# JuliaRobotics/KernelDensityEstimate.jl

Hardware: AMD Instinct MI355X
Metric: gibbs_product_samples_per_sec (higher is better)
Workload: dtype f64

## Files before the change

kerneldensityestimate.jl_amd/csrc/gibbs_lean.hip:

```cpp
#define KDEHIP_EXP256 1
#ifndef KDEHIP_PRELOAD_MAXB
#define KDEHIP_PRELOAD_MAXB 8
#endif
#include "gibbs_device.hpp"
#include "screen_device.hpp"

namespace kdehip {

template <int I> using IC = std::integral_constant<int, I>;
template <int N, int I = 0, typename F>
__device__ __forceinline__ void static_for(F &&f) {
  if constexpr (I < N) {
    f(IC<I>{});
    static_for<N, I + 1>(f);
  }
}

#if defined(KDEHIP_LEAN_HI) || (defined(KDEHIP_LEAN_DEV_M) && KDEHIP_LEAN_DEV_M > 4)
constexpr int kLeanMinDens = 8, kLeanMaxDens = 8;
#else
constexpr int kLeanMinDens = 2, kLeanMaxDens = 4;
#endif
constexpr int kLeanMaxNormals = 128;

__device__ __forceinline__ int scalar_copy(int x) {
  int y;
  asm("s_mov_b32 %0, %1" : "=s"(y) : "s"(x));
  return y;
}

template <int D>
struct LeanTile {
  int n;
  int flags;
  int lds_off;
  int stage_bytes;
  int chunk_rows;
  int seg;
  int hdr_lo, hdr_hi;
  int B, F, last_lane;
  int uniform_bw;
  __device__ __forceinline__ int64_t hdr_off() const {
    return (static_cast<int64_t>(hdr_hi) << 32) | static_cast<uint32_t>(hdr_lo);
  }
  __device__ __forceinline__ void load(const kdehip_v8i &d) {
    n = scalar_copy(d[0]);
    flags = scalar_copy(d[1]);
    lds_off = scalar_copy(d[2]);
    stage_bytes = scalar_copy(d[3]);
    chunk_rows = scalar_copy(d[4]);
    seg = scalar_copy(d[5]);
    hdr_lo = scalar_copy(d[6]);
    hdr_hi = scalar_copy(d[7]);
    B = (n + 63) >> 6;
    last_lane = flags & 0xFF;
    uniform_bw = flags >> 8;
    F = uniform_bw ? D + 1 : 2 * D + 1;
  }
};

template <typename P, typename T, bool OK> constexpr bool kCanPreloadImpl = OK && kIsLdsPtr<P> && sizeof(T) == 8;

template <typename T, int D, int M, int WAVES, bool BATCH = false, bool SCHUNK = false>
__global__ __launch_bounds__(WAVES * 64) void gibbs_lean_kernel(PlanDev plan_, RunArgs a_) {
  const LaunchView<BATCH> view(plan_, a_);
  const PlanDev &plan = view.plan;
  const auto &a = view.a;
  constexpr bool kPrefetchRows = (WAVES <= 12) || sizeof(T) == 4 || D <= 4;
  using RowPtr = std::conditional_t<(WAVES == 16 && sizeof(T) == 8), LdsPtrSplit<T>, LdsPtr<T>>;
  constexpr int kCopyWaves = WAVES > 4 ? 4 : WAVES;
  constexpr bool kKeptRows = (WAVES <= 8);
  constexpr bool kScreen = sizeof(T) == 8 && !BATCH;
  constexpr bool kPreloadBuild = kKeptRows && kPrefetchRows;
  constexpr int kNormOff = 2048;
  constexpr int kUnifOff = kNormOff + WAVES * kLeanMaxNormals * 8;
  constexpr int kPoolOff = kUnifOff + WAVES * 1024;
  constexpr bool kCoop = kScreen && SCHUNK && WAVES == 8;
  constexpr int kXchgOff = kPoolOff + kLdsPoolBytes;
  constexpr int kXchgSlotDoubles = 32 + 4 * 64;
  constexpr int kXchgBytes = kCoop ? 64 + WAVES * kXchgSlotDoubles * 8 : 0;
  static_assert(kPoolOff + kLdsPoolBytes + kXchgBytes <= 160 * 1024, "LDS budget of one CU exceeded");
  __shared__ __attribute__((aligned(1024))) unsigned char smem[kPoolOff + kLdsPoolBytes + kXchgBytes];

  double *sExpTab = reinterpret_cast<double *>(smem);
  if (threadIdx.x < 256) sExpTab[threadIdx.x] = kExp2Tab256[threadIdx.x];
  if constexpr (kCoop) {
    if (threadIdx.x < 16) reinterpret_cast<int *>(smem + kXchgOff)[threadIdx.x] = 0;
  }

  const int lane = threadIdx.x & 63;
  const int wave = __builtin_amdgcn_readfirstlane(static_cast<int>(threadIdx.x >> 6));
  KDEHIP_PRIO_CHAIN();
  const int chain = wave;
  int64_t s = static_cast<int64_t>(view.block) * WAVES + chain;
  const bool live = s < a.Np;
  if (!live) s = a.Np - 1;
  const uint64_t gs = static_cast<uint64_t>(a.sample_offset + s);
  const void *fb = live ? static_cast<const void *>(plan.levels) : nullptr;

  const int L = plan.L;
  const T *__restrict__ data = static_cast<const T *>(plan.data);
  const LevelTable levels{(const __attribute__((address_space(4))) kdehip_v16i *)(plan.levels)};
  const StepTable steps{(const __attribute__((address_space(4))) kdehip_v8i *)(plan.levels + 2 * plan.M * (plan.L + 1))};
  unsigned char *pool = smem + kPoolOff;
  const int dl = lane < D ? lane : D - 1;
  const int vlev = a.variant % 1000;

  double *sNorm = reinterpret_cast<double *>(smem + kNormOff) + chain * kLeanMaxNormals;
  const int R = D * (L + 1);
  if (a.rng_philox) {
    for (int b = lane; 2 * b < R; b += 64) {
      double n0, n1;
      philox_normal_pair(a.seed, gs, static_cast<uint32_t>(b), n0, n1);
      sNorm[2 * b] = n0;
      if (2 * b + 1 < R) sNorm[2 * b + 1] = n1;
    }
  } else {
    for (int r = lane; r < R; r += 64) sNorm[r] = a.randN[s * a.R + r];
  }
  __syncthreads();

  T lam[M], lmu[M];
  int psel[M];

  auto adopt = [&](auto jc, const auto &ds, auto hdr, int pos) {
    constexpr int j = decltype(jc)::value;
    using TA = TileAddr<T>;
    auto e = hdr + kTileHeader + TA::row(pos >> 6, TA::stride(ds.F)) + (pos & 63) * TA::kLane;
    const T mu = e[dl * TA::kField];
    const T var = ds.uniform_bw ? hdr[dl] : e[(D + dl) * TA::kField];
    const T l = fast_rcp(var);
    lam[j] = l;
    lmu[j] = mu * l;
    psel[j] = pos;
  };
  auto product = [&](auto skipc, T &mean, T &cov) {
    constexpr int skip = decltype(skipc)::value;
    T ls = T(0), ms = T(0);
    static_for<M>([&](auto kc) {
      constexpr int k = decltype(kc)::value;
      if constexpr (k != skip) { ls += lam[k]; ms += lmu[k]; }
    });
    cov = fast_rcp(ls);
    mean = cov * ms;
  };

  auto draw = [&](const auto &ds, auto hdr, T mean, T cov, auto &&run) -> int {
    if (ds.uniform_bw) {
      EvalUniform<T, D> ev;
      ev.tab = sExpTab;
      const T c = hdr[dl] + cov;
      T cen, nin;
      EvalUniform<T, D>::operands(mean, c, true, cen, nin);
      T Pr = T(1);
#pragma unroll
      for (int d = 0; d < D; ++d) {
        ev.center[d] = lane_read(cen, d);
        ev.ninv[d] = lane_read(nin, d);
        Pr *= lane_read(c, d);
      }
      ev.scale = Num<T>::rsqrt(Pr);
      return run(ev);
    }
    EvalFast<T, D, false> ev;
    ev.tab = sExpTab;
    ev.act = 0;
#pragma unroll
    for (int d = 0; d < D; ++d) {
      ev.center[d] = lane_read(mean, d);
      ev.cov[d] = lane_read(cov, d);
    }
    return run(ev);
  };

  uint32_t c = static_cast<uint32_t>(M);
  uint32_t ubatch = 0xFFFFFFFFu;
  double *sUnif = reinterpret_cast<double *>(smem + kUnifOff) + wave * 128;
  auto next_uniform = [&]() -> double {
    const uint32_t b = c >> 7;
    if (b != ubatch) {
      ubatch = b;
      double u_even, u_odd;
      if (a.rng_philox) {
        const Philox4 r = philox_block(a.seed, gs, b * 64u + static_cast<uint32_t>(lane), 0u);
        u_even = bits_to_unit(r.v[0], r.v[1]);
        u_odd = bits_to_unit(r.v[2], r.v[3]);
      } else {
        const int64_t i0 = s * a.K + static_cast<int64_t>(b) * 128 + 2 * lane - 1;
        u_even = (i0 >= 0 && i0 < a.nU) ? a.randU[i0] : 0.5;
        u_odd = (i0 + 1 < a.nU) ? a.randU[i0 + 1] : 0.5;
      }
      wave_sync();
      sUnif[2 * lane] = u_even;
      sUnif[2 * lane + 1] = u_odd;
      wave_sync();
    }
    const double u = sUnif[c & 127u];
    ++c;
    return u;
  };

  static_for<M>([&](auto jc) {
    const LevelDesc ds = levels[decltype(jc)::value * (L + 1)];
    adopt(jc, ds, data + ds.hdr_off, 0);
  });

  const TabTable tabs{(const __attribute__((address_space(4))) kdehip_v8i *)(plan.tabdesc)};
  const T *tables = static_cast<const T *>(plan.tables);
  const int Lt = (vlev == 1 || vlev == 4 || !a.use_tables) ? 0 : plan.Lt;

  auto draw_rows = [&](const auto &ds, auto rows, const auto &ev, double u) -> int {
    using P = decltype(rows);
    return draw_label<T, P, kPrefetchRows, kKeptRows>(rows, ds, lane, ev, u, fb);
  };

  auto draw_rows_repeat = [&](const auto &ds, const T *rows, const auto &ev, double u) -> int {
    using Ev = std::decay_t<decltype(ev)>;
    if constexpr (kScreen && SCHUNK && sizeof(typename Ev::Row) <= 7 * sizeof(T) && WAVES <= 8) {
      LaneAcc<T> acc;
      KDEHIP_PRIO_ROWS();
      lane_rows_all_deep<T, Ev>(rows, ds.B, TileAddr<T>::stride(ds.F), lane, ev, acc);
      KDEHIP_PRIO_CHAIN();
      return select_or_raise<T, const T *>(acc.total(), rows, ds, lane, ev, u, fb);
    }
    return draw_rows(ds, rows, ev, u);
  };

#ifdef KDEHIP_SCREEN_STAMPS
  unsigned long long rstamp[8] = {0, 0, 0, 0, 0, 0, 0, 0}, r_prev_end = 0;
  bool rstamp_on = false;
#define RSTAMP(var) const unsigned long long var = __builtin_amdgcn_s_memtime()
#define RSTAMP_ADD(slot, t0, t1) do { if (rstamp_on) rstamp[slot] += (t1) - (t0); } while (0)
#else
#define RSTAMP(var) do {} while (0)
#define RSTAMP_ADD(slot, t0, t1) do {} while (0)
#endif
  auto step_kept = [&](auto jc, const auto &ds, auto hdr, const auto &row, T mean, T cov, double u) {
    RSTAMP(tr1);
    auto rows1 = hdr + kTileHeader;
    using P1 = decltype(rows1);
    using Ev = EvalFast<T, D, false>;
    Ev ev;
    ev.tab = sExpTab;
    ev.act = 0;
#pragma unroll
    for (int d = 0; d < D; ++d) {
      ev.center[d] = lane_read(mean, d);
      ev.cov[d] = lane_read(cov, d);
    }
#ifdef KDEHIP_SCREEN_STAMPS
    asm volatile("" ::"s"(ev.center[D - 1]), "s"(ev.cov[D - 1]));
#endif
    RSTAMP(tr2);
    RSTAMP_ADD(1, tr1, tr2);
    int pos1;
    if (ds.B == 1) {
      const T S = ev(row);
      pos1 = select_or_raise<T, P1>(S, rows1, ds, lane, ev, u, fb);
    } else if (ds.B <= 4) {
      pos1 = draw_label_kept<T, P1, Ev, 4>(rows1, ds, lane, ev, u, fb, row);
    } else {
      pos1 = draw_label_kept<T, P1, Ev, 8>(rows1, ds, lane, ev, u, fb, row);
    }
    pos1 = __builtin_amdgcn_readfirstlane(pos1);
    RSTAMP(tr3);
    RSTAMP_ADD(2, tr2, tr3);
    adopt(jc, ds, hdr, pos1);
#ifdef KDEHIP_SCREEN_STAMPS
    {
      const double sink = lam[decltype(jc)::value] + lmu[decltype(jc)::value];
      asm volatile("" ::"v"(sink));
    }
#endif
    RSTAMP(tr4);
    RSTAMP_ADD(3, tr3, tr4);
#ifdef KDEHIP_SCREEN_STAMPS
    r_prev_end = tr4;
#endif
  };

  auto step = [&](auto jc, const auto &ds, auto hdr, bool first, T x) {
    if constexpr (kCanPreloadImpl<decltype(hdr + kTileHeader), T, kPreloadBuild>) {
      if (!ds.uniform_bw && ds.B <= KDEHIP_PRELOAD_MAXB) {
        RSTAMP(tr0);
#ifdef KDEHIP_SCREEN_STAMPS
        if (r_prev_end) RSTAMP_ADD(4, r_prev_end, tr0);
#endif
        const auto row = EvalFast<T, D, false>().load(hdr + kTileHeader + lane * TileAddr<T>::kLane);
        T mean1 = x, cov1 = T(0);
        if (!first) product(jc, mean1, cov1);
        const double u1 = next_uniform();
#ifdef KDEHIP_SCREEN_STAMPS
        asm volatile("" ::"v"(mean1), "v"(cov1), "v"(u1));
        {
          RSTAMP(trp);
          RSTAMP_ADD(0, tr0, trp);
        }
#endif
        step_kept(jc, ds, hdr, row, mean1, cov1, u1);
        return;
      }
    }
    T mean = x, cov = T(0);
    if (!first) product(jc, mean, cov);
    const double u = next_uniform();
    auto rows = hdr + kTileHeader;
    const int pos = __builtin_amdgcn_readfirstlane(draw(ds, hdr, mean, cov, [&](const auto &ev) {
      return draw_rows(ds, rows, ev, u);
    }));
    adopt(jc, ds, hdr, pos);
  };

  uint32_t n_screened = 0, n_repeated = 0;
#ifdef KDEHIP_SCREEN_STAMPS
  unsigned long long sstamp[8] = {0, 0, 0, 0, 0, 0, 0, 0};
  bool sstamp_on = false;
#endif
  auto screen_eval = [&](const auto &ds, double mu0, double cmin, float mmax, float valid, T mean, T cov, auto &&body) -> int {
    const float cen = static_cast<float>(mean - mu0);
    const float cf = static_cast<float>(cmin + cov), covf = static_cast<float>(cov);
    const float acen = fabsf(cen);
    const float t = fminf(mmax + acen, 2.0f * acen);
    float a2 = lane < D ? t * t * __builtin_amdgcn_rcpf(cf) : 0.0f;
    const bool inr = (acen <= kScreenMaxAbsMean) && (covf <= static_cast<float>(kScreenMaxVar)) && (a2 <= kScreenMaxA2);
    const bool ok = valid != 0.0f && __ballot(lane < D && !inr) == 0ull;
    a2 += dpp_fetch<0x111, 0xF>(a2);
    a2 += dpp_fetch<0x112, 0xF>(a2);
    a2 += dpp_fetch<0x114, 0xF>(a2);
    const float na = __builtin_sqrtf(lane_read(a2, 7)) * (kScreenU * kScreenSqrtC0 * 1.01f);
    using SC = ScreenConst<D>;
    const float Bc = (kScreenLn2 * 1.01f) * (na + (ds.uniform_bw ? SC::kx_uni : SC::kx_node) * kScreenU);
    const float A = (kScreenLn2 * 1.01f) * na +
                    (static_cast<float>(((ds.B + 1) >> 1) + 9) + (ds.uniform_bw ? SC::vc_uni : SC::vc_node)) * kScreenU;
    if (ds.uniform_bw) {
      ScreenEval<D, true> ev;
      ev.A = A; ev.Bc = Bc;
      const float ninv = -kScreenC0 * __builtin_amdgcn_rcpf(cf);
      float pr = 1.0f;
#pragma unroll
      for (int d = 0; d < D; ++d) {
        ev.cen[d] = lane_read(cen, d);
        ev.b[d] = lane_read(ninv, d);
        pr *= lane_read(cf, d);
      }
      ev.scale = __builtin_amdgcn_rsqf(pr);
      return body(ev, ok);
    } else {
      ScreenEval<D, false> ev;
      ev.A = A; ev.Bc = Bc; ev.scale = 1.0f;
#pragma unroll
      for (int d = 0; d < D; ++d) {
        ev.cen[d] = lane_read(cen, d);
        ev.b[d] = lane_read(covf, d);
      }
      return body(ev, ok);
    }
  };
  auto screen_finish = [&](auto jc, const auto &ds, int pos, T mean, T cov, double u) {
    const T *hdrg = data + ds.hdr_off();
    ++n_screened;
    if (pos < 0) {
      ++n_repeated;
      pos = __builtin_amdgcn_readfirstlane(draw(ds, hdrg, mean, cov, [&](const auto &ev) {
        return draw_rows_repeat(ds, hdrg + kTileHeader, ev, u);
      }));
    }
    adopt(jc, ds, hdrg, pos);
  };
  bool pend = false;
  T pend_mean = T(0), pend_cov = T(0);
  double pend_u = 0.0;
  int cstep = 0;
  auto coop_post = [&](T mean, T cov, double u) {
    if constexpr (kCoop) {
      pend = true; pend_mean = mean; pend_cov = cov; pend_u = u;
      double *xs = reinterpret_cast<double *>(smem + kXchgOff + 64) + wave * kXchgSlotDoubles;
      if (lane < D) { xs[dl] = static_cast<double>(mean); xs[8 + dl] = static_cast<double>(cov); }
      if (lane == 0) reinterpret_cast<int *>(smem + kXchgOff)[(cstep & 1) * WAVES + wave] = 1;
    }
  };
  auto coop_resolve = [&](auto jp, const auto &dsp, int par) {
    if constexpr (kCoop) {
      int *flags = reinterpret_cast<int *>(smem + kXchgOff) + par * WAVES;
      const int f = flags[lane & (WAVES - 1)];
      const unsigned mask = static_cast<unsigned>(__ballot(f != 0 && lane < WAVES));
      if (mask == 0u) return;
      using TA = TileAddr<T>;
      const T *hdrg = data + dsp.hdr_off();
      const T *rows = hdrg + kTileHeader;
      const int RS = TA::stride(dsp.F), B = dsp.B;
      const int group = wave >> 2, k = wave & 3;
      int idx = 0;
      for (unsigned m = mask; m != 0u; m &= m - 1u, ++idx) {
        if ((idx & 1) != group) continue;
        const int r = __builtin_ctz(m);
        double *xs = reinterpret_cast<double *>(smem + kXchgOff + 64) + r * kXchgSlotDoubles;
        const T mean_r = static_cast<T>(xs[dl]), cov_r = static_cast<T>(xs[8 + dl]);
        T acc = T(0);
        KDEHIP_PRIO_ROWS();
        draw(dsp, hdrg, mean_r, cov_r, [&](const auto &ev) {
          using Ev = std::decay_t<decltype(ev)>;
          using Row = typename Ev::Row;
          const T *e = rows + lane * TA::kLane;
          auto at = [&](int rr) { return e + TA::row(rr < B ? rr : B - 1, RS); };
          if constexpr (sizeof(Row) <= 4 * sizeof(T)) {
            Row a0 = ev.load(at(k)), a1 = ev.load(at(k + 4)), a2 = ev.load(at(k + 8)), a3 = ev.load(at(k + 12));
            int i = k;
            for (; i + 12 < B; i += 16) {
              const Row b0 = ev.load(at(i + 16)), b1 = ev.load(at(i + 20)), b2 = ev.load(at(i + 24)), b3 = ev.load(at(i + 28));
              __builtin_amdgcn_sched_barrier(0);
              acc += ev(a0); acc += ev(a1); acc += ev(a2); acc += ev(a3);
              a0 = b0; a1 = b1; a2 = b2; a3 = b3;
            }
            if (i < B) acc += ev(a0);
            if (i + 4 < B) acc += ev(a1);
            if (i + 8 < B) acc += ev(a2);
          } else {
            Row a0 = ev.load(at(k)), a1 = ev.load(at(k + 4));
            int i = k;
            for (; i + 4 < B; i += 8) {
              const Row b0 = ev.load(at(i + 8)), b1 = ev.load(at(i + 12));
              __builtin_amdgcn_sched_barrier(0);
              acc += ev(a0); acc += ev(a1);
              a0 = b0; a1 = b1;
            }
            if (i < B) acc += ev(a0);
          }
          return 0;
        });
        KDEHIP_PRIO_CHAIN();
        xs[32 + 64 * k + lane] = static_cast<double>(acc);
      }
      __syncthreads();
      if (pend) {
        double *xs = reinterpret_cast<double *>(smem + kXchgOff + 64) + wave * kXchgSlotDoubles;
        const T a0 = static_cast<T>(xs[32 + lane]), a1 = static_cast<T>(xs[32 + 64 + lane]);
        const T a2 = static_cast<T>(xs[32 + 128 + lane]), a3 = static_cast<T>(xs[32 + 192 + lane]);
        const T S = (a0 + a1) + (a2 + a3);
        const int pos = __builtin_amdgcn_readfirstlane(draw(dsp, hdrg, pend_mean, pend_cov, [&](const auto &ev) {
          return select_or_raise<T, const T *>(S, rows, dsp, lane, ev, pend_u, fb);
        }));
        adopt(jp, dsp, hdrg, pos);
        pend = false;
        if (lane == 0) flags[wave] = 0;
      }
    }
  };

  auto step_screen = [&](auto jc, const auto &ds, int sc_lds_off, bool first, T x) {
    if constexpr (kScreen) {
      SSTAMP(ts0);
      const LdsPtr<float> h32 = (LdsPtr<float>)(pool + sc_lds_off);
      const LdsPtr<double> h64 = (LdsPtr<double>)(pool + sc_lds_off);
      const double mu0 = h64[dl], cmin = h64[8 + dl];
      const float mmax = h32[32 + dl], valid = h32[40];
      T mean = x, cov = T(0);
      if (!first) product(jc, mean, cov);
      const double u = next_uniform();
      SSTAMP(ts1);
      SSTAMP_ADD(0, ts0, ts1);
      const float cen = static_cast<float>(mean - mu0);
      const float cf = static_cast<float>(cmin + cov), covf = static_cast<float>(cov);
      const float acen = fabsf(cen);
      const float t = fminf(mmax + acen, 2.0f * acen);
      float a2 = lane < D ? t * t * __builtin_amdgcn_rcpf(cf) : 0.0f;
      const bool inr = (acen <= kScreenMaxAbsMean) && (covf <= static_cast<float>(kScreenMaxVar)) && (a2 <= kScreenMaxA2);
      int pos = -1;
      const T *hdrg = data + ds.hdr_off();
      if (valid != 0.0f && __ballot(lane < D && !inr) == 0ull) {
        a2 += dpp_fetch<0x111, 0xF>(a2);
        a2 += dpp_fetch<0x112, 0xF>(a2);
        a2 += dpp_fetch<0x114, 0xF>(a2);
        const float na = __builtin_sqrtf(lane_read(a2, 7)) * (kScreenU * kScreenSqrtC0 * 1.01f);
        using SC = ScreenConst<D>;
        const float Bc = (kScreenLn2 * 1.01f) * (na + (ds.uniform_bw ? SC::kx_uni : SC::kx_node) * kScreenU);
        const float A = (kScreenLn2 * 1.01f) * na +
                        (static_cast<float>(((ds.B + 1) >> 1) + 9) + (ds.uniform_bw ? SC::vc_uni : SC::vc_node)) * kScreenU;
        const LdsPtr<float> rows32 = h32 + kScreenHeaderFloats;
        if (ds.uniform_bw) {
          ScreenEval<D, true> ev;
          ev.A = A; ev.Bc = Bc;
          const float ninv = -kScreenC0 * __builtin_amdgcn_rcpf(cf);
          float pr = 1.0f;
#pragma unroll
          for (int d = 0; d < D; ++d) {
            ev.cen[d] = lane_read(cen, d);
            ev.b[d] = lane_read(ninv, d);
            pr *= lane_read(cf, d);
          }
          ev.scale = __builtin_amdgcn_rsqf(pr);
          pos = screen_draw<D, true>(rows32, ds.n, ds.B, ds.F, lane, ev, u SSTAMP_ARGS);
        } else {
          ScreenEval<D, false> ev;
          ev.A = A; ev.Bc = Bc; ev.scale = 1.0f;
#pragma unroll
          for (int d = 0; d < D; ++d) {
            ev.cen[d] = lane_read(cen, d);
            ev.b[d] = lane_read(covf, d);
          }
          pos = screen_draw<D, false>(rows32, ds.n, ds.B, ds.F, lane, ev, u SSTAMP_ARGS);
        }
        pos = __builtin_amdgcn_readfirstlane(pos);
      }
      SSTAMP(ts2);
      SSTAMP_ADD(1, ts1, ts2);
      ++n_screened;
      if (pos < 0) {
        ++n_repeated;
        pos = __builtin_amdgcn_readfirstlane(draw(ds, hdrg, mean, cov, [&](const auto &ev) {
          return draw_rows_repeat(ds, hdrg + kTileHeader, ev, u);
        }));
      }
      SSTAMP(ts3);
      SSTAMP_ADD(2, ts2, ts3);
      adopt(jc, ds, hdrg, pos);
#ifdef KDEHIP_SCREEN_STAMPS
      {
        const double sink = lam[decltype(jc)::value] + lmu[decltype(jc)::value];
        asm volatile("" ::"v"(sink));
      }
#endif
      SSTAMP(ts4);
      SSTAMP_ADD(3, ts3, ts4);
    }
  };

  int gchunk = 0;
  auto stage_chunk = [&](const auto &ds, int r0, int half) {
    using TA = TileAddr<T>;
    const int RS = TA::stride(ds.F), rc = ds.chunk_rows;
    const int nrows = (ds.B - r0 < rc) ? (ds.B - r0) : rc;
    const int bytes = (static_cast<int>(TA::span(nrows, RS)) * int(sizeof(T)) + 1023) & ~1023;
    const unsigned char *src = reinterpret_cast<const unsigned char *>(data + ds.hdr_off() + kTileHeader + TA::row(r0, RS));
    if (wave < kCopyWaves) stage_tile<kCopyWaves>(src, pool + half * (kLdsPoolBytes / 2), bytes, wave, lane);
  };

  auto stage_schunk = [&](const LevelDesc &sc, int p0, int half) {
    using TA = TileAddr<float>;
    const int RS = TA::stride(sc.F), cp = sc.chunk_rows >> 1, npairs = (sc.B + 1) >> 1;
    const int np = (npairs - p0 < cp) ? (npairs - p0) : cp;
    const int head = p0 == 0 ? kScreenHeaderFloats : 0;
    const int bytes = ((head + np * RS) * 4 + 1023) & ~1023;
    const unsigned char *src = reinterpret_cast<const unsigned char *>(reinterpret_cast<const float *>(plan.data) + sc.hdr_off +
                                                                       (p0 == 0 ? 0 : kScreenHeaderFloats + p0 * RS));
    if (wave < kCopyWaves) stage_tile<kCopyWaves>(src, pool + half * (kLdsPoolBytes / 2), bytes, wave, lane);
  };
  auto step_screen_chunked = [&](auto jc, const auto &ds, const auto &dsp, const LevelDesc &sc, const LevelDesc &scn, bool more,
                                 bool first, bool level_start, T x) {
    if constexpr (kScreen && SCHUNK) {
      using TA = TileAddr<float>;
      T mean = x, cov = T(0);
      const bool was_pend = kCoop && pend;
      if (!first && !was_pend) product(jc, mean, cov);
      const double u = next_uniform();
      const int RS = TA::stride(sc.F), cp = sc.chunk_rows >> 1, npairs = (sc.B + 1) >> 1;
      staging_barrier();
      if (cp < npairs) stage_schunk(sc, cp, (gchunk + 1) & 1);
      else if (more) stage_schunk(scn, 0, (gchunk + 1) & 1);
      if constexpr (kCoop) {
        constexpr int j = decltype(jc)::value;
        if (!level_start) coop_resolve(IC<(j + M - 1) % M>{}, dsp, (cstep + 1) & 1);
        if (was_pend && !first) product(jc, mean, cov);
      }
      const LdsPtr<float> h32 = (LdsPtr<float>)(pool + (gchunk & 1) * (kLdsPoolBytes / 2));
      const LdsPtr<double> h64 = (LdsPtr<double>)(pool + (gchunk & 1) * (kLdsPoolBytes / 2));
      const double mu0 = h64[dl], cmin = h64[8 + dl];
      const float mmax = h32[32 + dl], valid = h32[40];
      const float *grows = reinterpret_cast<const float *>(plan.data) + sc.hdr_off + kScreenHeaderFloats;
      const int pos = __builtin_amdgcn_readfirstlane(screen_eval(ds, mu0, cmin, mmax, valid, mean, cov, [&](const auto &ev, bool ok) {
        using Ev = std::decay_t<decltype(ev)>;
        ScreenSums q;
        KDEHIP_PRIO_ROWS();
        if (ok) screen_rows<D, Ev::kUni>(h32 + kScreenHeaderFloats + lane * TA::kLane, npairs < cp ? npairs : cp, RS, ev, q);
        ++gchunk;
        for (int p0 = cp; p0 < npairs; p0 += cp, ++gchunk) {
          staging_barrier();
          if (p0 + cp < npairs) stage_schunk(sc, p0 + cp, (gchunk + 1) & 1);
          else if (more) stage_schunk(scn, 0, (gchunk + 1) & 1);
          const int np = (npairs - p0 < cp) ? (npairs - p0) : cp;
          if (ok) screen_rows<D, Ev::kUni>((LdsPtr<float>)(pool + (gchunk & 1) * (kLdsPoolBytes / 2)) + lane * TA::kLane, np, RS, ev, q);
        }
        KDEHIP_PRIO_CHAIN();
        if (!ok) return -1;
        return screen_decide<D, Ev::kUni, true>(grows, ds.n, ds.B, RS, lane, ev, u, q.values(), q.errors() SSTAMP_ARGS);
      }));
      if constexpr (kCoop) {
        ++n_screened;
        if (pos < 0) {
          ++n_repeated;
          coop_post(mean, cov, u);
        } else {
          adopt(jc, ds, data + ds.hdr_off(), pos);
        }
        ++cstep;
      } else {
        screen_finish(jc, ds, pos, mean, cov, u);
      }
    }
  };

#ifdef KDEHIP_EXPERIMENTS
  const int Lrun = (vlev >= 100 && vlev - 100 < L) ? vlev - 100 : L;
#else
  const int Lrun = L;
#endif
  for (int l = 1; l <= Lrun; ++l) {
    T x;
    {
      T mean, cov;
      product(IC<-1>{}, mean, cov);
      x = mean + Num<T>::sqrt(cov) * static_cast<T>(sNorm[(l - 1) * D + dl]);
    }
    const int level_mode = scalar_copy(levels[l].stage_mode);
    auto tile_raw = [&](int j) -> kdehip_v8i { return steps.raw(j * (L + 1) + l); };
    auto tile = [&](int j) -> LeanTile<D> {
      LeanTile<D> t;
      t.load(tile_raw(j));
      return t;
    };
    const int mode = vlev == 1 ? int(kStageGlobal) : level_mode;
    const bool tabulated = (l <= Lt);
    const int npass = tabulated ? 1 : a.Niter + 1;

    bool screened = false, screen_streamed = false, screen_chunked = false;
    if constexpr (kScreen) {
      if (a.use_screen && vlev != 1) {
        const int smode = scalar_copy(levels[M * (L + 1) + l].stage_mode);
        screened = smode == kStageScreen;
        screen_streamed = smode == kStageScreenStream;
        if constexpr (SCHUNK) screen_chunked = smode == kStageScreenChunked;
      }
    }
#ifdef KDEHIP_SCREEN_STAMPS
    rstamp_on = (vlev >= 300 && l == vlev - 300) && view.block == 3 && wave == 5;
    r_prev_end = 0;
#endif
    if (screened) {
#ifdef KDEHIP_SCREEN_STAMPS
      sstamp_on = (l == ((vlev >= 200) ? vlev - 200 : L)) && view.block == 3 && wave == 5;
#endif
      auto screen = [&](int j) -> LevelDesc { return levels[(M + j) * (L + 1) + l]; };
      staging_barrier();
      static_for<M>([&](auto jc) {
        const LevelDesc sc = screen(decltype(jc)::value);
        stage_tile<WAVES>(reinterpret_cast<const unsigned char *>(reinterpret_cast<const float *>(plan.data) + sc.hdr_off),
                          pool + sc.lds_off, sc.stage_bytes, wave, lane);
      });
      staging_barrier();
      for (int p = 0; p < npass; ++p)
        static_for<M>([&](auto jc) {
          const LeanTile<D> ds = tile(decltype(jc)::value);
          step_screen(jc, ds, ds.lds_off, p == 0, x);
        });
    } else if (screen_streamed) {
      auto screen = [&](int j) -> LevelDesc { return levels[(M + j) * (L + 1) + l]; };
      auto stage_screen = [&](const LevelDesc &sc, int half, auto wc) {
        constexpr int W = decltype(wc)::value;
        if (wave < W)
          stage_tile<W>(reinterpret_cast<const unsigned char *>(reinterpret_cast<const float *>(plan.data) + sc.hdr_off),
                        pool + half * (kLdsPoolBytes / 2), sc.stage_bytes, wave, lane);
      };
      staging_barrier();
      stage_screen(screen(0), 0, IC<WAVES>{});
      int t = 0;
      const int nsteps = npass * M;
      for (int p = 0; p < npass; ++p)
        static_for<M>([&](auto jc) {
          constexpr int j = decltype(jc)::value;
          constexpr int jn = (j + 1 == M) ? 0 : j + 1;
          const LeanTile<D> ds = tile(j);
          const LevelDesc scn = screen(jn);
          staging_barrier();
          constexpr bool kLateCopy = kCopyWaves < WAVES;
          if (!kLateCopy && t + 1 < nsteps) stage_screen(scn, (t + 1) & 1, IC<WAVES>{});
          step_screen(jc, ds, (t & 1) * (kLdsPoolBytes / 2), p == 0, x);
          if (kLateCopy && t + 1 < nsteps) stage_screen(scn, (t + 1) & 1, IC<kCopyWaves>{});
          ++t;
        });
    } else if (screen_chunked) {
      auto screen = [&](int j) -> LevelDesc { return levels[(M + j) * (L + 1) + l]; };
      staging_barrier();
      stage_schunk(screen(0), 0, gchunk & 1);
      int t = 0;
      const int nsteps = npass * M;
      for (int p = 0; p < npass; ++p)
        static_for<M>([&](auto jc) {
          constexpr int j = decltype(jc)::value;
          constexpr int jn = (j + 1 == M) ? 0 : j + 1;
          constexpr int jp = (j + M - 1) % M;
          const LeanTile<D> ds = tile(j);
          step_screen_chunked(jc, ds, tile(jp), screen(j), screen(jn), t + 1 < nsteps, p == 0, t == 0, x);
          ++t;
        });
      if constexpr (kCoop) {
        __syncthreads();
        coop_resolve(IC<M - 1>{}, tile(M - 1), (cstep + 1) & 1);
      }
    } else if (mode == kStageResident) {
      staging_barrier();
      static_for<M>([&](auto jc) {
        const LeanTile<D> ds = tile(decltype(jc)::value);
        stage_tile<WAVES>(reinterpret_cast<const unsigned char *>(data + ds.hdr_off()), pool + ds.lds_off, ds.stage_bytes, wave, lane);
      });
      staging_barrier();
      for (int p = 0; p < npass; ++p)
        static_for<M>([&](auto jc) {
          const LeanTile<D> ds = tile(decltype(jc)::value);
          step(jc, ds, (RowPtr)(pool + ds.lds_off), p == 0, x);
        });
    } else if (mode == kStageStream) {
      staging_barrier();
      {
        const LeanTile<D> d0 = tile(0);
        stage_tile<WAVES>(reinterpret_cast<const unsigned char *>(data + d0.hdr_off()), pool, d0.stage_bytes, wave, lane);
      }
      int t = 0;
      const int nsteps = npass * M;
      for (int p = 0; p < npass; ++p)
        static_for<M>([&](auto jc) {
          constexpr int j = decltype(jc)::value;
          constexpr int jn = (j + 1 == M) ? 0 : j + 1;
          const LeanTile<D> ds = tile(j);
          const LeanTile<D> dn = tile(jn);
          T mean = x, cov = T(0);
          if (p != 0) product(jc, mean, cov);
          const double u = next_uniform();
          staging_barrier();
          constexpr bool kLateCopy = kCopyWaves < WAVES;
          if (!kLateCopy && t + 1 < nsteps)
            stage_tile<WAVES>(reinterpret_cast<const unsigned char *>(data + dn.hdr_off()),
                              pool + ((t + 1) & 1) * (kLdsPoolBytes / 2), dn.stage_bytes, wave, lane);
          {
            auto hdr = (RowPtr)(pool + (t & 1) * (kLdsPoolBytes / 2));
            auto rows = hdr + kTileHeader;
            const int pos = __builtin_amdgcn_readfirstlane(draw(ds, hdr, mean, cov, [&](const auto &ev) {
              return draw_rows(ds, rows, ev, u);
            }));
            adopt(jc, ds, hdr, pos);
          }
          if (kLateCopy && t + 1 < nsteps && wave < kCopyWaves)
            stage_tile<kCopyWaves>(reinterpret_cast<const unsigned char *>(data + dn.hdr_off()),
                                   pool + ((t + 1) & 1) * (kLdsPoolBytes / 2), dn.stage_bytes, wave, lane);
          ++t;
        });
    } else if (mode == kStageChunked) {
      staging_barrier();
      stage_chunk(tile(0), 0, gchunk & 1);
      int t = 0;
      const int nsteps = npass * M;
      for (int p = 0; p < npass; ++p)
        static_for<M>([&](auto jc) {
          constexpr int j = decltype(jc)::value;
          constexpr int jn = (j + 1 == M) ? 0 : j + 1;
          const LeanTile<D> ds = tile(j);
          const LeanTile<D> dn = tile(jn);
          T mean = x, cov = T(0);
          if (p != 0) product(jc, mean, cov);
          const double u = next_uniform();
          const T *hdr = data + ds.hdr_off();
          const int pos = draw(ds, hdr, mean, cov, [&](const auto &ev) {
            using Ev = std::decay_t<decltype(ev)>;
            const int RS = TileAddr<T>::stride(ds.F), rc = ds.chunk_rows;
            LaneAcc<T> acc;
            SegSums<T> seg;
            const int cps = seg_chunks(ds.seg);
            const bool use_seg = cps != 0;
            int cin = 0;
            KDEHIP_PRIO_ROWS();
            for (int r0 = 0; r0 < ds.B; r0 += rc, ++gchunk) {
              staging_barrier();
              if (r0 + rc < ds.B) stage_chunk(ds, r0 + rc, (gchunk + 1) & 1);
              else if (t + 1 < nsteps) stage_chunk(dn, 0, (gchunk + 1) & 1);
              const int nrows = (ds.B - r0 < rc) ? (ds.B - r0) : rc;
              const auto crows = (RowPtr)(pool + (gchunk & 1) * (kLdsPoolBytes / 2));
              lane_rows_all<T, RowPtr, Ev, kPrefetchRows>(crows, nrows, RS, lane, ev, acc);
              if (use_seg && ++cin == cps) { seg.note(acc.total()); cin = 0; }
            }
            KDEHIP_PRIO_CHAIN();
            const T S = acc.total();
            if (use_seg)
              return __builtin_amdgcn_readfirstlane(
                  select_or_raise_seg<T, const T *>(S, seg, cps * rc, hdr + kTileHeader, ds, lane, ev, u, fb));
            return __builtin_amdgcn_readfirstlane(select_or_raise<T, const T *>(S, hdr + kTileHeader, ds, lane, ev, u, fb));
          });
          adopt(jc, ds, hdr, pos);
          ++t;
        });
    } else {
      for (int p = 0; p < npass; ++p)
        static_for<M>([&](auto jc) {
          const LeanTile<D> ds = tile(decltype(jc)::value);
          step(jc, ds, data + ds.hdr_off(), p == 0, x);
        });
    }

    if (tabulated) {
      TabDesc td[M];
      static_for<M>([&](auto jc) { td[decltype(jc)::value] = tabs[decltype(jc)::value * (L + 1) + l]; });
      uint32_t word = 0;
      static_for<M>([&](auto jc) { word |= static_cast<uint32_t>(psel[decltype(jc)::value]) << td[decltype(jc)::value].shift; });
      word = __builtin_amdgcn_readfirstlane(word);
      for (int p = 1; p <= a.Niter; ++p)
        static_for<M>([&](auto jc) {
          constexpr int j = decltype(jc)::value;
          const TabDesc &tj = td[j];
          const uint32_t cfg = (word & ((1u << tj.shift) - 1u)) | ((word >> (tj.shift + tj.bits)) << tj.shift);
          const T *row = tables + tj.off + static_cast<int64_t>(cfg) * (tj.n + 1);
          const int n = tj.n;
          const T incl = row[lane < n ? lane : n];
          const double u = next_uniform();
          const T total = lane_read(incl, n < 64 ? n : 63);
          int pos;
          if (!(total >= Num<T>::tiny_total())) {
            count_fallback(fb, lane);
            const LeanTile<D> dk = tile(j);
            const T wl = ((LdsPtr<T>)(pool + dk.lds_off) + kTileHeader)[(dk.F - 1) * TileAddr<T>::kField + (n - 1) * TileAddr<T>::kLane];
            int z = n - 1;
            if (wl > T(0)) {
              z = static_cast<int>(ceil(u * static_cast<double>(n))) - 1;
              z = z < 0 ? 0 : (z > n - 1 ? n - 1 : z);
            }
            pos = __builtin_amdgcn_readfirstlane(z);
          } else {
            const T target = static_cast<T>(u) * total;
            unsigned long long hit = __ballot(target <= incl);
            if (n < 64) hit &= (1ull << n) - 1ull;
            pos = hit ? (__ffsll(hit) - 1) : (n - 1);
          }
          word = (word & ~(((1u << tj.bits) - 1u) << tj.shift)) | (static_cast<uint32_t>(pos) << tj.shift);
        });
      static_for<M>([&](auto jc) {
        constexpr int j = decltype(jc)::value;
        const int pk = static_cast<int>((word >> td[j].shift) & ((1u << td[j].bits) - 1u));
        const LeanTile<D> dk = tile(j);
        adopt(jc, dk, (LdsPtr<T>)(pool + dk.lds_off), pk);
      });
    }
    if (a.labels && live && lane == 0) {
      static_for<M>([&](auto jc) {
        constexpr int j = decltype(jc)::value;
        a.labels[(s * M + j) * L + (l - 1)] = plan.perm[levels[j * (L + 1) + l].perm_off + psel[j]];
      });
    }
    if (l == L && live && lane == 0) {
      static_for<M>([&](auto jc) {
        constexpr int j = decltype(jc)::value;
        const int64_t label = static_cast<int64_t>(plan.perm[levels[j * (L + 1) + l].perm_off + psel[j]]) + 1;
        a.indices[s * M + j] = label;
        for (int k = 0; k < a.npeers; ++k) a.peer_indices[k][s * M + j] = label;
      });
    }
  }

#ifdef KDEHIP_SCREEN_STAMPS
  if (view.block == 3 && wave == 5 && lane == 0)
    for (int k = 0; k < 8; ++k) { g_screen_stamps[k] = sstamp[k]; g_screen_stamps[8 + k] = rstamp[k]; }
#endif
  if constexpr (kScreen) {
    if (live && lane == 0 && n_screened != 0u) {
      unsigned long long *cnt = reinterpret_cast<unsigned long long *>(const_cast<LevelDesc *>(plan.levels));
      atomicAdd(cnt - 3, static_cast<unsigned long long>(n_screened));
      if (n_repeated != 0u) atomicAdd(cnt - 2, static_cast<unsigned long long>(n_repeated));
    }
  }
  {
    T mean, cov;
    product(IC<-1>{}, mean, cov);
    T xf = mean;
    if (a.addEntropy) xf = mean + Num<T>::sqrt(cov) * static_cast<T>(sNorm[L * D + dl]);
    if (live && lane < D) {
      a.points[s * D + lane] = static_cast<double>(xf);
      for (int k = 0; k < a.npeers; ++k) a.peer_points[k][s * D + lane] = static_cast<double>(xf);
    }
  }
}


template <typename T, int D, int M, int WAVES>
static void launch_lean_waves(const PlanDev &plan, const RunArgs &args, hipStream_t stream) {
  const int64_t blocks = (args.Np + WAVES - 1) / WAVES;
  if constexpr (sizeof(T) == 8 && WAVES >= 8) {
    if (M == 8 || (plan.screened == 2 && args.use_screen)) {
      hipLaunchKernelGGL((gibbs_lean_kernel<T, D, M, WAVES, false, true>), dim3(static_cast<unsigned>(blocks)), dim3(WAVES * 64),
                         0, stream, plan, args);
      return;
    }
  }
  if constexpr (!(sizeof(T) == 8 && WAVES >= 8 && M == 8))
    hipLaunchKernelGGL((gibbs_lean_kernel<T, D, M, WAVES>), dim3(static_cast<unsigned>(blocks)), dim3(WAVES * 64), 0,
                       stream, plan, args);
}

static int set_geometry(const PlanDev &, RunArgs &args, int) { return lean_waves(args.Np, args.variant); }

template <typename T, int D, int M>
static int launch_lean_m(const PlanDev &plan, const RunArgs &args_in, hipStream_t stream) {
  RunArgs args = args_in;
  const int waves = set_geometry(plan, args, sizeof(T) == 8 ? 64 : 32);
  if (waves == 16) launch_lean_waves<T, D, M, 16>(plan, args, stream);
  else if (waves == 8) launch_lean_waves<T, D, M, 8>(plan, args, stream);
  else launch_lean_waves<T, D, M, 4>(plan, args, stream);
  const hipError_t e = hipGetLastError();
  if (e != hipSuccess)
    return set_error(KDEHIP_ERR_HIP, std::string("kernel launch failed: ") + hipGetErrorString(e));
  return KDEHIP_OK;
}

#ifndef KDEHIP_DIM
#error "compile gibbs_lean.hip with -DKDEHIP_DIM=<1..8>"
#endif
#define KDEHIP_CAT2(a, b) a##b
#define KDEHIP_CAT(a, b) KDEHIP_CAT2(a, b)

template <typename T, int D, int M>
static int launch_lean_m_hi(const PlanDev &plan, const RunArgs &args_in, hipStream_t stream) {
  RunArgs args = args_in;
  const int waves = set_geometry(plan, args, sizeof(T) == 8 ? 64 : 32);
  if (waves == 16) launch_lean_waves<T, D, M, 16>(plan, args, stream);
  else if (waves == 8) launch_lean_waves<T, D, M, 8>(plan, args, stream);
  else return kLeanNotCovered;
  const hipError_t e = hipGetLastError();
  if (e != hipSuccess)
    return set_error(KDEHIP_ERR_HIP, std::string("kernel launch failed: ") + hipGetErrorString(e));
  return KDEHIP_OK;
}

#if !defined(KDEHIP_LEAN_HI) && !defined(KDEHIP_LEAN_F32) && !defined(KDEHIP_LEAN_DEV)
template <int D, int M>
static void launch_lean_batch_m(const PlanDev &plan, const RunArgs &args, hipStream_t stream) {
  constexpr int W = 16;
  hipLaunchKernelGGL((gibbs_lean_kernel<double, D, M, W, true>), dim3(static_cast<unsigned>(args.Np / W)), dim3(W * 64), 0,
                     stream, plan, args);
}
int KDEHIP_CAT(launch_lean_batch_d, KDEHIP_DIM)(int M, const PlanDev &plan, const RunArgs &args, void *stream) {
  constexpr int D = KDEHIP_DIM;
  hipStream_t st = static_cast<hipStream_t>(stream);
  if (args.Np <= 0) return KDEHIP_OK;
  switch (M) {
    case 2: launch_lean_batch_m<D, 2>(plan, args, st); break;
    case 3: launch_lean_batch_m<D, 3>(plan, args, st); break;
    case 4: launch_lean_batch_m<D, 4>(plan, args, st); break;
    default: return set_error(KDEHIP_ERR_UNSUPPORTED, "batched launch: 2..4 densities");
  }
  const hipError_t e = hipGetLastError();
  if (e != hipSuccess) return set_error(KDEHIP_ERR_HIP, std::string("batched kernel launch failed: ") + hipGetErrorString(e));
  return KDEHIP_OK;
}
#endif

#if defined(KDEHIP_LEAN_DEV) && !defined(KDEHIP_LEAN_HI) && !defined(KDEHIP_LEAN_F32)
int KDEHIP_CAT(launch_lean_batch_d, KDEHIP_DIM)(int, const PlanDev &, const RunArgs &, void *) {
  return set_error(KDEHIP_ERR_UNSUPPORTED, "development library: no batched kernels");
}
#endif

#if defined(KDEHIP_SCREEN_STAMPS)
extern "C" int kdehip_debug_read_screen_stamps(unsigned long long *out) {
  return hipMemcpyFromSymbol(out, HIP_SYMBOL(kdehip::g_screen_stamps), sizeof(unsigned long long) * 16) == hipSuccess ? 0 : -5;
}
#endif

#if defined(KDEHIP_LEAN_HI)
#define KDEHIP_LEAN_ENTRY launch_lean_hi_d
#elif defined(KDEHIP_LEAN_F32)
#define KDEHIP_LEAN_ENTRY launch_lean_f32_d
#else
#define KDEHIP_LEAN_ENTRY launch_lean_d
#endif

int KDEHIP_CAT(KDEHIP_LEAN_ENTRY, KDEHIP_DIM)(int precision, int mode, const PlanDev &plan, const RunArgs &args,
                                              void *stream) {
  constexpr int D = KDEHIP_DIM;
  if (mode != kModeFast || args.table_build || plan.M < kLeanMinDens || plan.M > kLeanMaxDens ||
      D * (plan.L + 1) > kLeanMaxNormals)
    return kLeanNotCovered;
  if (args.Np <= 0) return KDEHIP_OK;
  hipStream_t st = static_cast<hipStream_t>(stream);
  const bool f64 = (precision == 64);
#ifdef KDEHIP_LEAN_DEV
#ifndef KDEHIP_LEAN_DEV_M
#define KDEHIP_LEAN_DEV_M 4
#endif
#ifndef KDEHIP_LEAN_DEV_W
#define KDEHIP_LEAN_DEV_W 8
#endif
#ifdef KDEHIP_LEAN_DEV_F32
  using DevT = float;
#else
  using DevT = double;
#endif
  RunArgs dargs = args;
  if (f64 != (sizeof(DevT) == 8) || plan.M != KDEHIP_LEAN_DEV_M ||
      set_geometry(plan, dargs, precision) != KDEHIP_LEAN_DEV_W)
    return kLeanNotCovered;
  launch_lean_waves<DevT, D, KDEHIP_LEAN_DEV_M, KDEHIP_LEAN_DEV_W>(plan, dargs, st);
  return KDEHIP_OK;
#elif defined(KDEHIP_LEAN_HI)
  if (!f64) return kLeanNotCovered;
  return launch_lean_m_hi<double, D, 8>(plan, args, st);
#elif defined(KDEHIP_LEAN_F32)
  if (f64) return kLeanNotCovered;
  switch (plan.M) {
    case 2: return launch_lean_m<float, D, 2>(plan, args, st);
    case 3: return launch_lean_m<float, D, 3>(plan, args, st);
    default: return launch_lean_m<float, D, 4>(plan, args, st);
  }
#else
  if (!f64) return kLeanNotCovered;
  switch (plan.M) {
    case 2: return launch_lean_m<double, D, 2>(plan, args, st);
    case 3: return launch_lean_m<double, D, 3>(plan, args, st);
    default: return launch_lean_m<double, D, 4>(plan, args, st);
  }
#endif
}

}
```

Before: 4.276 million.

## Pair consecutive tabulated Gibbs updates to prefetch conditional rows speculatively

In the tabulated Gibbs loop, consecutive density updates are now processed in pairs. For the second density, all candidate table rows (one per possible choice of the first density) are loaded up front into registers before the first selection is known. The intent is to remove the serial dependency between the first selection and the second density's global load, hiding memory latency. In exchange it issues extra loads and ballots, uses more registers, and only applies when the product of the two sizes fits in 256 entries; odd M needs a tail path.

New measurement: 4.117 million. 3.7% lower.

```diff
diff --git a/kerneldensityestimate.jl_amd/csrc/gibbs_lean.hip b/kerneldensityestimate.jl_amd/csrc/gibbs_lean.hip
--- a/kerneldensityestimate.jl_amd/csrc/gibbs_lean.hip
+++ b/kerneldensityestimate.jl_amd/csrc/gibbs_lean.hip
@@ -800,35 +800,104 @@
       uint32_t word = 0;
       static_for<M>([&](auto jc) { word |= static_cast<uint32_t>(psel[decltype(jc)::value]) << td[decltype(jc)::value].shift; });
       word = __builtin_amdgcn_readfirstlane(word);
-      for (int p = 1; p <= a.Niter; ++p)
-        static_for<M>([&](auto jc) {
-          constexpr int j = decltype(jc)::value;
-          const TabDesc &tj = td[j];
-          const uint32_t cfg = (word & ((1u << tj.shift) - 1u)) | ((word >> (tj.shift + tj.bits)) << tj.shift);
-          const T *row = tables + tj.off + static_cast<int64_t>(cfg) * (tj.n + 1);
-          const int n = tj.n;
-          const T incl = row[lane < n ? lane : n];
-          const double u = next_uniform();
-          const T total = lane_read(incl, n < 64 ? n : 63);
-          int pos;
-          if (!(total >= Num<T>::tiny_total())) {
-            count_fallback(fb, lane);
-            const LeanTile<D> dk = tile(j);
-            const T wl = ((LdsPtr<T>)(pool + dk.lds_off) + kTileHeader)[(dk.F - 1) * TileAddr<T>::kField + (n - 1) * TileAddr<T>::kLane];
-            int z = n - 1;
-            if (wl > T(0)) {
-              z = static_cast<int>(ceil(u * static_cast<double>(n))) - 1;
-              z = z < 0 ? 0 : (z > n - 1 ? n - 1 : z);
+      constexpr int kTabPairRegs = 4;
+      auto tab_fallback = [&](auto jc, int n, double u) -> int {
+        count_fallback(fb, lane);
+        const LeanTile<D> dk = tile(decltype(jc)::value);
+        const T wl = ((LdsPtr<T>)(pool + dk.lds_off) + kTileHeader)[(dk.F - 1) * TileAddr<T>::kField + (n - 1) * TileAddr<T>::kLane];
+        int z = n - 1;
+        if (wl > T(0)) {
+          z = static_cast<int>(ceil(u * static_cast<double>(n))) - 1;
+          z = z < 0 ? 0 : (z > n - 1 ? n - 1 : z);
+        }
+        return __builtin_amdgcn_readfirstlane(z);
+      };
+      auto tab_select = [&](auto jc, int n, T incl, double u) -> int {
+        const T total = lane_read(incl, n < 64 ? n : 63);
+        if (!(total >= Num<T>::tiny_total())) return tab_fallback(jc, n, u);
+        const T target = static_cast<T>(u) * total;
+        unsigned long long hit = __ballot(target <= incl);
+        if (n < 64) hit &= (1ull << n) - 1ull;
+        return hit ? (__ffsll(hit) - 1) : (n - 1);
+      };
+      auto tab_row = [&](const TabDesc &tj, uint32_t w) -> const T * {
+        const uint32_t cfg = (w & ((1u << tj.shift) - 1u)) | ((w >> (tj.shift + tj.bits)) << tj.shift);
+        return tables + tj.off + static_cast<int64_t>(cfg) * (tj.n + 1);
+      };
+      auto tab_single = [&](auto jc) {
+        constexpr int j = decltype(jc)::value;
+        const TabDesc &tj = td[j];
+        const int n = tj.n;
+        const T incl = tab_row(tj, word)[lane < n ? lane : n];
+        const double u = next_uniform();
+        const int pos = tab_select(jc, n, incl, u);
+        word = (word & ~(((1u << tj.bits) - 1u) << tj.shift)) | (static_cast<uint32_t>(pos) << tj.shift);
+      };
+      auto tab_pair = [&](auto jc) {
+        constexpr int j = decltype(jc)::value;
+        constexpr int jn = (j + 1) % M;
+        const TabDesc &tj = td[j];
+        const TabDesc &tn = td[jn];
+        const int nj = tj.n, nn = tn.n;
+        const double u0 = next_uniform();
+        const double u1 = next_uniform();
+        const T incl0 = tab_row(tj, word)[lane < nj ? lane : nj];
+        const T *row1 = tab_row(tn, word & ~(((1u << tj.bits) - 1u) << tj.shift));
+        const int hstride = (nn + 1) << (tj.shift < tn.shift ? tj.shift : tj.shift - tn.bits);
+        const int nv = nj * nn;
+        T val[kTabPairRegs];
+#pragma unroll
+        for (int k = 0; k < kTabPairRegs; ++k) {
+          val[k] = T(0);
+          if (k * 64 < nv) {
+            const int v = k * 64 + lane;
+            val[k] = row1[((v >> tn.bits) & (nj - 1)) * hstride + (v & (nn - 1))];
+          }
+        }
+        const T tot1 = row1[(lane & (nj - 1)) * hstride + nn];
+        const int pos0 = tab_select(jc, nj, incl0, u0);
+        const T total1 = lane_read(tot1, pos0);
+        int pos1;
+        if (!(total1 >= Num<T>::tiny_total())) {
+          pos1 = tab_fallback(IC<jn>{}, nn, u1);
+        } else {
+          const T target1 = static_cast<T>(u1) * total1;
+          const int v0 = pos0 << tn.bits;
+          unsigned long long hit = 0ull;
+#pragma unroll
+          for (int k = 0; k < kTabPairRegs; ++k) {
+            if (k * 64 < nv) {
+              const unsigned long long hk = __ballot(target1 <= val[k]);
+              if ((v0 >> 6) == k) hit = hk;
             }
-            pos = __builtin_amdgcn_readfirstlane(z);
-          } else {
-            const T target = static_cast<T>(u) * total;
-            unsigned long long hit = __ballot(target <= incl);
-            if (n < 64) hit &= (1ull << n) - 1ull;
-            pos = hit ? (__ffsll(hit) - 1) : (n - 1);
           }
-          word = (word & ~(((1u << tj.bits) - 1u) << tj.shift)) | (static_cast<uint32_t>(pos) << tj.shift);
-        });
+          hit >>= (v0 & 63);
+          if (nn < 64) hit &= (1ull << nn) - 1ull;
+          pos1 = hit ? (__ffsll(hit) - 1) : (nn - 1);
+        }
+        word = (word & ~((((1u << tj.bits) - 1u) << tj.shift) | (((1u << tn.bits) - 1u) << tn.shift))) |
+               (static_cast<uint32_t>(pos0) << tj.shift) | (static_cast<uint32_t>(pos1) << tn.shift);
+      };
+      bool pairable = true;
+      static_for<M>([&](auto jc) {
+        constexpr int j = decltype(jc)::value;
+        if (td[j].n * td[(j + 1) % M].n > 64 * kTabPairRegs) pairable = false;
+      });
+      if (pairable) {
+        constexpr int kUnitPasses = (M % 2 == 0) ? 1 : 2;
+        constexpr int kUnitPairs = kUnitPasses * M / 2;
+        int p = a.Niter;
+        for (; p >= kUnitPasses; p -= kUnitPasses)
+          static_for<kUnitPairs>([&](auto qc) { tab_pair(IC<(2 * decltype(qc)::value) % M>{}); });
+        if constexpr (M % 2 == 1) {
+          if (p > 0) {
+            static_for<M / 2>([&](auto qc) { tab_pair(IC<2 * decltype(qc)::value>{}); });
+            tab_single(IC<M - 1>{});
+          }
+        }
+      } else {
+        for (int p = 1; p <= a.Niter; ++p) static_for<M>([&](auto jc) { tab_single(jc); });
+      }
       static_for<M>([&](auto jc) {
         constexpr int j = decltype(jc)::value;
         const int pk = static_cast<int>((word >> td[j].shift) & ((1u << td[j].bits) - 1u));
```
